# HeyWeCome/WhisprRec

Hardware: AMD Instinct MI355X
Metric: BPR training triplets/sec (higher is better)
Workload: dtype f32; 1 GPU; BPRMF emb_size=64, synthetic 1000000 users x 1000000 items (uniform ids), batch 65536, SGD l2=0, plan build in timed region; batch=65536, emb_size=64, optimizer=SGD, plan_chunk_batches=64, tables=single GPU, step_stream=whisprrec_amd.hip_ops.PipelinedSgd, plan=group plan (no per-batch sort: flags + lists of the shared rows, wr_group.hip), chained_step_launch=True, plan_build=on a side stream, beside the steps of the chunk before

## Files before the change

include/whisprrec_hip.h:

```cpp
#ifndef WHISPRREC_HIP_H
#define WHISPRREC_HIP_H

#include <stdint.h>

#ifdef __cplusplus
extern "C" {
#endif

#define WR_ABI_VERSION 1

#define WR_OK 0
#define WR_E_NULL (-1)
#define WR_E_SHAPE (-2)
#define WR_E_WORKSPACE (-3)
#define WR_E_ALIGN (-4)
#define WR_E_RANGE (-5)

int32_t wr_abi_version(void);
const char *wr_last_error(void);
int32_t wr_device_info(int32_t *n_cu, int32_t *wave_size, char *arch, int32_t arch_len);

int64_t wr_bpr_fwd_workspace_bytes(int64_t B);
int32_t wr_bpr_fwd(const float *user_tab, int64_t n_users, const float *item_tab, int64_t n_items, int32_t D,
                   const int64_t *u, const int64_t *p, const int64_t *n, int64_t B, float *pos_score, float *neg_score,
// ... 127 lines not shown
                          int64_t workspace_bytes, void *stream);

int32_t wr_bprmf_run_sgd(float *user_tab, int64_t n_users, float *item_tab, int64_t n_items, int32_t D,
                         const int32_t *tu, const int32_t *tp, const int32_t *tn, const int32_t *oc_item,
                         const int32_t *oc_src, int64_t n_triplets, int64_t batch_size, int64_t first_batch,
                         int64_t n_batches, float lr, float *loss_out, void *const *phase_events, const wr_hot_runs *hot,
                         void *workspace, int64_t workspace_bytes, void *stream);

int32_t wr_bprmf_chain_supported(const float *user_tab, const float *item_tab, int32_t D);
int64_t wr_bprmf_chain_sync_words(int64_t n_batches);
int32_t wr_bprmf_run_sgd_chain(float *user_tab, int64_t n_users, float *item_tab, int64_t n_items, int32_t D,
                               const int32_t *tu, const int32_t *tp, const int32_t *tn, const int32_t *oc_item,
                               const int32_t *oc_src, int64_t n_triplets, int64_t batch_size, int64_t first_batch,
                               int64_t n_batches, float lr, float *loss_out, const int32_t *tdef, const int32_t *def_q,
                               const int32_t *def_count_host, int64_t def_cap, int64_t def_limit, void *const *phase_events,
                               void *workspace, int64_t workspace_bytes, int32_t *sync, int64_t sync_words, void *stream);

int64_t wr_group_plan_words(int64_t n_triplets, int64_t batch_size, int64_t n_users, int64_t n_items);
int32_t wr_group_plan_layout(int64_t n_triplets, int64_t batch_size, int64_t n_users, int64_t n_items, int64_t *out);
int32_t wr_narrow_ids_i64(const int64_t *u, const int64_t *p, const int64_t *n, int32_t *u32, int32_t *p32, int32_t *n32,
                          int64_t count, void *stream);
int32_t wr_group_plan_build(const int32_t *u, const int32_t *p, const int32_t *n, int64_t n_triplets, int64_t batch_size,
                            int64_t n_users, int64_t n_items, int32_t *plan, int64_t plan_words, void *stream);
int64_t wr_bprmf_group_workspace_bytes(int64_t batch_size, int32_t D);
int64_t wr_bprmf_group_sync_words(int64_t n_batches);
int32_t wr_bprmf_group_supported(const float *user_tab, const float *item_tab, int32_t D);
int32_t wr_bprmf_run_sgd_group(float *user_tab, int64_t n_users, float *item_tab, int64_t n_items, int32_t D,
                               const int32_t *u, const int32_t *p, const int32_t *n, int64_t n_triplets, int64_t batch_size,
                               const int32_t *plan, int64_t plan_words, int64_t first_batch, int64_t n_batches, float lr,
                               float *loss_out, void *const *events, void *workspace, int64_t workspace_bytes, int32_t *sync,
                               int64_t sync_words, void *stream);

int32_t wr_bprmf_plan_overlap_marks(const int32_t *tu, const int32_t *tp, const int32_t *tn, int64_t n_triplets,
                                    int64_t batch_size, int64_t n_items, const int32_t *prev_bitmap, int32_t *bitmap,
                                    int32_t *tdef, int32_t *def_q, int64_t def_cap, int32_t *def_count, void *stream);

int32_t wr_bprmf_plan_overlap_deferred(const int32_t *tu, const int32_t *tp, const int32_t *tn, int64_t n_triplets,
                                       int64_t batch_size, int64_t n_items, const int32_t *prev_bitmap, const int32_t *bitmap,
                                       int32_t *tdef, int32_t *def_q, int64_t def_cap, int32_t *def_count, void *stream);

int32_t wr_bprmf_grads(const float *user_tab, int64_t n_users, const float *item_tab, int64_t n_items, int32_t D,
                       const int32_t *tu, const int32_t *tp, const int32_t *tn, const int32_t *oc_item,
                       const int32_t *oc_src, int64_t B, float *grad_u, float *grad_i, int32_t *stamp_u,
                       int32_t *stamp_i, int32_t step_id, float *loss_out, const wr_hot_runs *hot, void *workspace,
                       int64_t workspace_bytes, void *stream);

// ... 208 lines not shown
```

whisprrec_amd/abi.py:

```python
import ctypes
import os

_HERE = os.path.dirname(os.path.abspath(__file__))
LIB_PATH = os.path.join(_HERE, "libwhisprrec_hip.so")

c_i32, c_i64, c_f32, c_vp = ctypes.c_int32, ctypes.c_int64, ctypes.c_float, ctypes.c_void_p

SIGNATURES = {
    "wr_abi_version": (c_i32, []),
    "wr_last_error": (ctypes.c_char_p, []),
    "wr_device_info": (c_i32, [c_vp, c_vp, c_vp, c_i32]),
    "wr_bpr_fwd_workspace_bytes": (c_i64, [c_i64]),
    "wr_bpr_fwd": (c_i32, [c_vp, c_i64, c_vp, c_i64, c_i32, c_vp, c_vp, c_vp, c_i64, c_vp, c_vp, c_vp, c_vp, c_vp, c_i64,
                           c_vp]),
    "wr_bprmf_plan_workspace_bytes": (c_i64, [c_i64, c_i64, c_i64, c_i64]),
    "wr_bprmf_plan_build_i64": (c_i32, [c_vp, c_vp, c_vp, c_i64, c_i64, c_i64, c_i64, c_vp, c_vp, c_vp, c_vp, c_vp, c_vp,
                                        c_vp, c_vp, c_i64, c_vp]),
    "wr_bprmf_plan_build_i32": (c_i32, [c_vp, c_vp, c_vp, c_i64, c_i64, c_i64, c_i64, c_vp, c_vp, c_vp, c_vp, c_vp, c_vp,
                                        c_vp, c_vp, c_i64, c_vp]),
    "wr_bprmf_plan_small_max_batch": (c_i64, []),
    "wr_bprmf_plan_build_small_i64": (c_i32, [c_vp, c_vp, c_vp, c_i64, c_i64, c_i64, c_i64, c_vp, c_vp, c_vp, c_vp, c_vp, c_vp,
                                              c_vp, c_vp]),
    "wr_bprmf_plan_build_small_i32": (c_i32, [c_vp, c_vp, c_vp, c_i64, c_i64, c_i64, c_i64, c_vp, c_vp, c_vp, c_vp, c_vp, c_vp,
                                              c_vp, c_vp]),
# ... 35 lines not shown
    "wr_bprmf_hot_caps": (None, [c_i64, c_i32, c_vp, c_vp]),
    "wr_bprmf_plan_hot_runs": (c_i32, [c_vp, c_i32, c_i64, c_i64, c_vp, c_vp, c_vp, c_vp, c_vp, c_vp, c_vp]),
    "wr_bprmf_step_sgd": (c_i32, [c_vp, c_i64, c_vp, c_i64, c_i32, c_vp, c_vp, c_vp, c_vp, c_vp, c_i64, c_f32, c_f32,
                                  c_vp, c_vp, c_i32, c_vp, c_vp, c_vp, c_i64, c_vp]),
    "wr_bprmf_run_sgd": (c_i32, [c_vp, c_i64, c_vp, c_i64, c_i32, c_vp, c_vp, c_vp, c_vp, c_vp, c_i64, c_i64, c_i64,
                                 c_i64, c_f32, c_vp, c_vp, c_vp, c_vp, c_i64, c_vp]),
    "wr_bprmf_chain_supported": (c_i32, [c_vp, c_vp, c_i32]),
    "wr_bprmf_chain_sync_words": (c_i64, [c_i64]),
    "wr_bprmf_run_sgd_chain": (c_i32, [c_vp, c_i64, c_vp, c_i64, c_i32, c_vp, c_vp, c_vp, c_vp, c_vp, c_i64, c_i64, c_i64,
                                       c_i64, c_f32, c_vp, c_vp, c_vp, c_vp, c_i64, c_i64, c_vp, c_vp, c_i64, c_vp, c_i64,
                                       c_vp]),
    "wr_lightgcn_step_workspace_bytes": (c_i64, [c_i64, c_i64, c_i32, c_i64, c_i64]),
    "wr_lightgcn_step": (c_i32, [c_vp, c_vp, c_i64, c_i64, c_i32, c_i64, c_vp, c_vp, c_vp, c_vp, c_i32, c_i32, c_vp, c_vp, c_vp,
                                 c_i64, c_f32, c_i32, c_vp, c_vp, c_vp, c_vp, c_i64, c_vp]),
    "wr_shard_route": (c_i32, [c_vp, c_vp, c_vp, c_i64, c_i64, c_i32, c_i32, c_i64, c_i64, c_i64, c_i64, c_i64, c_vp, c_vp, c_vp,
                               c_vp, c_vp, c_vp, c_vp]),
    "wr_shard_pack": (c_i32, [c_vp, c_vp, c_i64, c_i32, c_i64, c_i64, c_vp, c_i64, c_vp, c_vp, c_vp]),
    "wr_bprmf_shard_step_group": (c_i32, [c_vp, c_i64, c_vp, c_i64, c_i64, c_i32, c_vp, c_vp, c_vp, c_i64, c_i64, c_vp, c_i64,
                                          c_i64, c_i64, c_f32, c_vp, c_vp, c_vp, c_i64, c_vp, c_i64, c_vp]),
    "wr_group_plan_words": (c_i64, [c_i64, c_i64, c_i64, c_i64]),
    "wr_group_plan_layout": (c_i32, [c_i64, c_i64, c_i64, c_i64, c_vp]),
    "wr_narrow_ids_i64": (c_i32, [c_vp, c_vp, c_vp, c_vp, c_vp, c_vp, c_i64, c_vp]),
    "wr_group_plan_build": (c_i32, [c_vp, c_vp, c_vp, c_i64, c_i64, c_i64, c_i64, c_vp, c_i64, c_vp]),
    "wr_bprmf_group_workspace_bytes": (c_i64, [c_i64, c_i32]),
    "wr_bprmf_group_sync_words": (c_i64, [c_i64]),
    "wr_bprmf_group_supported": (c_i32, [c_vp, c_vp, c_i32]),
    "wr_bprmf_run_sgd_group": (c_i32, [c_vp, c_i64, c_vp, c_i64, c_i32, c_vp, c_vp, c_vp, c_i64, c_i64, c_vp, c_i64, c_i64,
                                       c_i64, c_f32, c_vp, c_vp, c_vp, c_i64, c_vp, c_i64, c_vp]),
    "wr_bprmf_plan_overlap_deferred": (c_i32, [c_vp, c_vp, c_vp, c_i64, c_i64, c_i64, c_vp, c_vp, c_vp, c_vp, c_i64, c_vp,
                                               c_vp]),
    "wr_bprmf_plan_fast_marks_supported": (c_i32, [c_i64, c_i64, c_i64, c_i64]),
    "wr_bprmf_plan_build_fast_marks_i64": (c_i32, [c_vp, c_vp, c_vp, c_i64, c_i64, c_i64, c_i64, c_vp, c_vp, c_vp, c_vp, c_vp,
                                                   c_vp, c_vp, c_vp, c_i64, c_vp, c_vp]),
    "wr_bprmf_plan_build_fast_marks_i32": (c_i32, [c_vp, c_vp, c_vp, c_i64, c_i64, c_i64, c_i64, c_vp, c_vp, c_vp, c_vp, c_vp,
                                                   c_vp, c_vp, c_vp, c_i64, c_vp, c_vp]),
    "wr_bprmf_plan_overlap_marks": (c_i32, [c_vp, c_vp, c_vp, c_i64, c_i64, c_i64, c_vp, c_vp, c_vp, c_vp, c_i64, c_vp,
                                            c_vp]),
    "wr_bprmf_grads": (c_i32, [c_vp, c_i64, c_vp, c_i64, c_i32, c_vp, c_vp, c_vp, c_vp, c_vp, c_i64, c_vp, c_vp, c_vp,
                               c_vp, c_i32, c_vp, c_vp, c_vp, c_i64, c_vp]),
    "wr_sgd_decay_untouched": (c_i32, [c_vp, c_i64, c_i32, c_vp, c_i32, c_f32, c_f32, c_vp]),
    "wr_sgd_dense": (c_i32, [c_vp, c_i64, c_i32, c_vp, c_vp, c_i32, c_f32, c_f32, c_vp]),
    "wr_adam_dense": (c_i32, [c_vp, c_vp, c_vp, c_i64, c_i32, c_vp, c_vp, c_i32, c_i64, c_f32, c_f32, c_f32, c_f32,
                              c_f32, c_vp]),
    "wr_adam_dense_dev": (c_i32, [c_vp, c_vp, c_vp, c_i64, c_i32, c_vp, c_vp, c_i64, c_vp, c_f32, c_f32, c_f32, c_f32, c_vp]),
    "wr_adam_dense_dev_pair": (c_i32, [c_vp, c_vp, c_vp, c_i64, c_vp, c_vp, c_vp, c_vp, c_i64, c_vp, c_i32, c_vp, c_i64, c_vp,
                                       c_f32, c_f32, c_f32, c_f32, c_vp]),
# ... 133 lines not shown
```

whisprrec_amd/csrc/wr_group.hip:

```cpp
#include "wr_common.h"
#include <hip/hip_ext.h>

#include <algorithm>

namespace wr {

constexpr int kGpThreads = 1024;
constexpr unsigned kGpRangeBits = 18;
constexpr int kGpWords = 1 << (kGpRangeBits - 5);
constexpr int kGpCap = 8192;
constexpr int kGpBins = 4096;
constexpr int kGpMaxBin = 256;
constexpr int kGpMaxRanges = 8;
constexpr int64_t kGpMaxBatch = 1 << 17;
constexpr int kGpLongRun = 64;
constexpr int kGpMetaWords = 16;
#ifndef WR_GP_DBG
#define WR_GP_DBG 0
#endif

struct GroupLayout {
    int64_t nb, B, fw;
    int R_u, R_i, cap_u, cap_i;
    unsigned mask_u, mask_i, hbits_u, hbits_i;
    int64_t flags, ucnt, icnt, ul_row, ul_src, il_row, il_src, total;
    int64_t zero_words;
};

static inline int ranges_for(int64_t n_rows, unsigned *mask, unsigned *hbits, int *cap) {
    unsigned bits = kGpRangeBits;
    while (bits < kGpRangeBits + 3 && (int64_t(1) << bits) < n_rows) ++bits;
    *mask = (1u << bits) - 1u;
    *hbits = bits;
    const int R = 1 << (bits - kGpRangeBits);
    *cap = kGpCap;
    return R;
}

static bool group_layout(int64_t n, int64_t B, int64_t n_users, int64_t n_items, GroupLayout &L) {
    if (n <= 0 || n >= (int64_t(1) << 31) || B <= 0 || B > kGpMaxBatch) return false;
    if (n_users <= 0 || n_users >= (int64_t(1) << 31) || n_items <= 0 || n_items >= (int64_t(1) << 31)) return false;
    L.nb = (n + B - 1) / B;
    L.B = B;
    L.fw = (B + 31) / 32;
    L.R_u = ranges_for(n_users, &L.mask_u, &L.hbits_u, &L.cap_u);
    L.R_i = ranges_for(n_items, &L.mask_i, &L.hbits_i, &L.cap_i);
    L.flags = kGpMetaWords;
    L.ucnt = L.flags + L.nb * L.fw * 4;
    L.icnt = L.ucnt + align_up(L.nb * L.R_u, 4);
    L.zero_words = L.icnt + align_up(L.nb * L.R_i, 4);
    L.ul_row = L.zero_words;
    L.ul_src = L.ul_row + L.nb * L.R_u * (int64_t)L.cap_u;
    L.il_row = L.ul_src + L.nb * L.R_u * (int64_t)L.cap_u;
    L.il_src = L.il_row + L.nb * L.R_i * (int64_t)L.cap_i;
    L.total = L.il_src + L.nb * L.R_i * (int64_t)L.cap_i;
    return true;
}

struct GpDev {
    int *meta;
    unsigned *flags;
    int *ucnt, *icnt;
    int *ul_row, *ul_src, *il_row, *il_src;
    int R_u, R_i, cap_u, cap_i;
    unsigned mask_u, mask_i, hbits_u, hbits_i;
    int fw;
};

static inline GpDev group_dev(int32_t *plan, const GroupLayout &L) {
    return GpDev{plan, reinterpret_cast<unsigned *>(plan + L.flags), plan + L.ucnt, plan + L.icnt, plan + L.ul_row,
                 plan + L.ul_src, plan + L.il_row, plan + L.il_src, L.R_u, L.R_i, L.cap_u, L.cap_i, L.mask_u, L.mask_i,
                 L.hbits_u, L.hbits_i, (int)L.fw};
}

template <typename F>
__device__ __forceinline__ void gp_scan(const int *__restrict__ a, int cnt, F f) {
    if ((reinterpret_cast<uintptr_t>(a) & 15u) == 0) {
        const int n4 = cnt >> 2;
        const int4 *a4 = reinterpret_cast<const int4 *>(a);
        int i = threadIdx.x;
        for (; i + 3 * kGpThreads < n4; i += 4 * kGpThreads) {
            int4 v[4];
#pragma unroll
            for (int q = 0; q < 4; ++q) v[q] = a4[i + q * kGpThreads];
#pragma unroll
            for (int q = 0; q < 4; ++q) {
                const int at = 4 * (i + q * kGpThreads);
                f(v[q].x, at);
                f(v[q].y, at + 1);
                f(v[q].z, at + 2);
                f(v[q].w, at + 3);
            }
        }
        for (; i < n4; i += kGpThreads) {
            const int4 v = a4[i];
            f(v.x, 4 * i);
            f(v.y, 4 * i + 1);
            f(v.z, 4 * i + 2);
            f(v.w, 4 * i + 3);
        }
        for (int j = (n4 << 2) + threadIdx.x; j < cnt; j += kGpThreads) f(a[j], j);
    } else {
        for (int j = threadIdx.x; j < cnt; j += kGpThreads) f(a[j], j);
    }
}

__global__ __launch_bounds__(kGpThreads) void group_plan_kernel(const int *__restrict__ u, const int *__restrict__ p,
                                                                 const int *__restrict__ n, int64_t n_total, int B, int nb,
                                                                 int n_users, int n_items, GpDev L) {
    extern __shared__ __attribute__((aligned(16))) unsigned gp_lds[];
    unsigned *seen = gp_lds;
    unsigned long long *keys = reinterpret_cast<unsigned long long *>(gp_lds);
    unsigned *multi = gp_lds + 2 * kGpCap;
    unsigned *f0 = multi + kGpWords, *f1 = f0 + L.fw, *f2 = f1 + L.fw;
    int &n_list = *reinterpret_cast<int *>(f2 + L.fw);
    const int per = L.R_u + L.R_i;
    const unsigned lb = xcd_contiguous_id(blockIdx.x, gridDim.x);
    const int b = (int)(lb / (unsigned)per), rr = (int)(lb % (unsigned)per);
    const bool item = rr >= L.R_u;
    const unsigned r = (unsigned)(item ? rr - L.R_u : rr);
    const int64_t base = (int64_t)b * B;
    const int Bb = (int)((base + B <= n_total) ? B : (n_total - base));
    const unsigned n_rows = (unsigned)(item ? n_items : n_users);
    const unsigned mask = item ? L.mask_i : L.mask_u;
    const unsigned rb = (item ? L.hbits_i : L.hbits_u) - kGpRangeBits, rsel = (1u << rb) - 1u;
    for (int i = threadIdx.x; i < kGpWords; i += kGpThreads) {
        seen[i] = 0u;
        multi[i] = 0u;
    }
    for (int i = threadIdx.x; i < 3 * L.fw; i += kGpThreads) f0[i] = 0u;
    if (threadIdx.x == 0) n_list = 0;
    __syncthreads();
    auto mark = [&](int row, int) {
        if ((unsigned)row >= n_rows) {
            L.meta[0] = 1;
            return;
        }
        const unsigned h = (unsigned)row & mask;
        if ((h & rsel) != r) return;
        const unsigned bit = h >> rb, m = 1u << (bit & 31u);
        const unsigned old = atomicOr(&seen[bit >> 5], m);
        if (old & m) atomicOr(&multi[bit >> 5], m);
    };
    if (!(WR_GP_DBG & 8)) {
        if (item) {
            gp_scan(p + base, Bb, mark);
            gp_scan(n + base, Bb, mark);
        } else {
            gp_scan(u + base, Bb, mark);
        }
    }
    __syncthreads();
    auto several = [&](int row) -> bool {
        const unsigned h = (unsigned)row & mask;
        if ((h & rsel) != r) return false;
        const unsigned bit = h >> rb;
        return (multi[bit >> 5] >> (bit & 31u)) & 1u;
    };
    auto append = [&](int row, unsigned src) {
        const int pos = atomicAdd(&n_list, 1);
        if (pos < kGpCap) keys[pos] = ((unsigned long long)(unsigned)row << 32) | src;
    };
    if (!(WR_GP_DBG & 2)) {
        const bool next = b + 1 < nb && !(WR_GP_DBG & 16);
        const int64_t nbase = base + B;
        const int Bn = next ? (int)((nbase + B <= n_total) ? B : (n_total - nbase)) : 0;
        auto defer = [&](int row, int t) {
            if (several(row)) atomicOr(&f2[t >> 5], 1u << (t & 31));
        };
        if (item) {
            gp_scan(p + base, Bb, [&](int row, int t) {
                if (several(row)) {
                    atomicOr(&f0[t >> 5], 1u << (t & 31));
                    append(row, (unsigned)t << 1);
                }
            });
            gp_scan(n + base, Bb, [&](int row, int t) {
                if (several(row)) {
                    atomicOr(&f1[t >> 5], 1u << (t & 31));
                    append(row, ((unsigned)t << 1) | 1u);
                }
            });
            gp_scan(p + nbase, Bn, defer);
            gp_scan(n + nbase, Bn, defer);
        } else {
            gp_scan(u + base, Bb, [&](int row, int t) {
                if (several(row)) {
                    atomicOr(&f0[t >> 5], 1u << (t & 31));
                    append(row, (unsigned)t << 1);
                }
            });
            gp_scan(u + nbase, Bn, defer);
        }
// ... 54 lines not shown
            const int bin = bin_of(k);
            const int lo = bin ? cnt[bin - 1] : 0, hi = cnt[bin];
            if (hi - lo > kGpMaxBin) {
                L.meta[1] = 1;
                continue;
            }
            int pos = lo, same = 0;
            for (int jj = lo; jj < hi; ++jj) {
                const unsigned long long o = keys[out16[jj]];
                pos += o < k ? 1 : 0;
                same += (unsigned)(o >> 32) == (unsigned)(k >> 32) ? 1 : 0;
            }
            if (same > kGpLongRun) L.meta[2] = 1;
            lrow[pos] = (int)(k >> 32);
            lsrc[pos] = (int)(unsigned)k;
        }
    } else {
        for (int j = threadIdx.x; j < m; j += kGpThreads) {
            lrow[j] = (int)(keys[j] >> 32);
            lsrc[j] = (int)(unsigned)keys[j];
        }
    }
    if (threadIdx.x == 0) (item ? L.icnt : L.ucnt)[(int64_t)b * R + r] = m;
}

__global__ __launch_bounds__(kBlock) void narrow_ids_kernel(const int64_t *__restrict__ u, const int64_t *__restrict__ p,
                                                             const int64_t *__restrict__ n, int *__restrict__ u32,
                                                             int *__restrict__ p32, int *__restrict__ n32, int64_t cnt) {
    const int64_t i = (int64_t)blockIdx.x * kBlock + threadIdx.x;
    if (i >= cnt) return;
    const int64_t a = u[i], b = p[i], c = n[i];
    u32[i] = (a >= 0 && a < (int64_t(1) << 31)) ? (int)a : -1;
    p32[i] = (b >= 0 && b < (int64_t(1) << 31)) ? (int)b : -1;
    n32[i] = (c >= 0 && c < (int64_t(1) << 31)) ? (int)c : -1;
}

constexpr int kGsTile = 32;
constexpr int kGsAhead = 8;
constexpr int kGsShards = 64;
constexpr int kGsShardStride = 16;
constexpr int kGsStepWords = kGsShards * kGsShardStride;
constexpr int kGsDefChunk = 32;
constexpr int kGsLdsInts = 1024 + 8;
constexpr unsigned kGsSpinLimit = 1u << 22;

struct GsBatch {
// ... 468 lines not shown
        a.tiles_at = (int)((int64_t)a.nA * WR_GS_TILES_AT / 16);
        a.side_at = std::max(a.tiles_at, (int)((int64_t)a.nA * WR_GS_SIDE_AT / 16));
        const dim3 grid((unsigned)(a.nA + a.nIT + a.nUT + a.nDS));
        hipEvent_t e0 = have_cur ? ev(k, 0) : nullptr, e1 = have_cur ? ev(k, 1) : nullptr;
        if (e0 != nullptr || e1 != nullptr)
            hipExtLaunchKernelGGL((bprmf_group_step<T, NV, FULL>), grid, dim3(kBlock), 0, stream, e0, e1, 0, a);
        else
            hipLaunchKernelGGL((bprmf_group_step<T, NV, FULL>), grid, dim3(kBlock), 0, stream, a);
        WR_LAUNCH_CHECK("bprmf_group_step");
        n_partials_prev = a.nA + a.nDS;
    }
    return WR_OK;
}

}

using namespace wr;

extern "C" {

int64_t wr_group_plan_words(int64_t n_triplets, int64_t batch_size, int64_t n_users, int64_t n_items) {
    GroupLayout L;
    if (!group_layout(n_triplets, batch_size, n_users, n_items, L)) return 0;
    return L.total;
}

int32_t wr_group_plan_layout(int64_t n_triplets, int64_t batch_size, int64_t n_users, int64_t n_items, int64_t *out) {
    WR_REQUIRE(out != nullptr, WR_E_NULL, "out is NULL");
    GroupLayout L;
    WR_REQUIRE(group_layout(n_triplets, batch_size, n_users, n_items, L), WR_E_RANGE,
               "group plan not applicable to n=%lld, batch=%lld", (long long)n_triplets, (long long)batch_size);
    const int64_t v[16] = {L.nb, L.fw, L.R_u, L.R_i, (int64_t)L.mask_u, (int64_t)L.mask_i, L.flags, L.ucnt, L.icnt, L.ul_row,
                           L.ul_src, L.il_row, L.il_src, L.total, L.cap_u, L.cap_i};
    for (int i = 0; i < 16; ++i) out[i] = v[i];
    return WR_OK;
}

int32_t wr_narrow_ids_i64(const int64_t *u, const int64_t *p, const int64_t *n, int32_t *u32, int32_t *p32, int32_t *n32,
                          int64_t count, void *stream_) {
    WR_REQUIRE(u && p && n && u32 && p32 && n32, WR_E_NULL, "index arrays must not be NULL");
    WR_REQUIRE(count >= 0 && count < (int64_t(1) << 40), WR_E_SHAPE, "count out of range");
    if (count == 0) return WR_OK;
    hipLaunchKernelGGL(narrow_ids_kernel, dim3((unsigned)((count + kBlock - 1) / kBlock)), dim3(kBlock), 0,
                       reinterpret_cast<hipStream_t>(stream_), u, p, n, u32, p32, n32, count);
    WR_LAUNCH_CHECK("narrow_ids_kernel");
    return WR_OK;
}

int32_t wr_group_plan_build(const int32_t *u, const int32_t *p, const int32_t *n, int64_t n_triplets, int64_t batch_size,
                            int64_t n_users, int64_t n_items, int32_t *plan, int64_t plan_words, void *stream_) {
    WR_REQUIRE(u && p && n && plan, WR_E_NULL, "index arrays / plan must not be NULL");
    GroupLayout L;
    WR_REQUIRE(group_layout(n_triplets, batch_size, n_users, n_items, L), WR_E_RANGE,
               "group plan not applicable to n=%lld, batch=%lld", (long long)n_triplets, (long long)batch_size);
    WR_REQUIRE(aligned16(plan) && plan_words >= L.total, WR_E_WORKSPACE, "group plan: %lld words < %lld", (long long)plan_words,
               (long long)L.total);
    WR_REQUIRE(L.nb * (L.R_u + L.R_i) < (int64_t(1) << 31), WR_E_SHAPE, "group plan: too many batches in one plan");
    hipStream_t stream = reinterpret_cast<hipStream_t>(stream_);
    WR_HIP(hipMemsetAsync(plan, 0, (size_t)L.zero_words * 4, stream));
    const size_t lds = (size_t)(2 * kGpCap + kGpWords + 3 * L.fw + 4) * 4;
    static bool attr_set = false;
    if (!attr_set) {
        WR_HIP(hipFuncSetAttribute(reinterpret_cast<const void *>(group_plan_kernel), hipFuncAttributeMaxDynamicSharedMemorySize,
                                   (int)((2 * kGpCap + kGpWords + 3 * ((kGpMaxBatch + 31) / 32) + 4) * 4)));
        attr_set = true;
    }
    const GpDev G = group_dev(plan, L);
    hipLaunchKernelGGL(group_plan_kernel, dim3((unsigned)(L.nb * (L.R_u + L.R_i))), dim3(kGpThreads), lds, stream, u, p, n,
                       n_triplets, (int)batch_size, (int)L.nb, (int)n_users, (int)n_items, G);
    WR_LAUNCH_CHECK("group_plan_kernel");
    return WR_OK;
}

int64_t wr_bprmf_group_workspace_bytes(int64_t batch_size, int32_t D) { return 2 * gs_ws_one(batch_size, D); }

int64_t wr_bprmf_group_sync_words(int64_t n_batches) { return n_batches < 0 ? WR_E_SHAPE : (n_batches + 1) * kGsStepWords + 4; }

int32_t wr_bprmf_group_supported(const float *user_tab, const float *item_tab, int32_t D) {
    return (user_tab && item_tab && D >= 4 && D <= 1024 && D % 4 == 0 && gs_shape_ok(user_tab, item_tab, D)) ? 1 : 0;
}

int32_t wr_bprmf_run_sgd_group(float *user_tab, int64_t n_users, float *item_tab, int64_t n_items, int32_t D,
                               const int32_t *u, const int32_t *p, const int32_t *n, int64_t n_triplets, int64_t batch_size,
                               const int32_t *plan, int64_t plan_words, int64_t first_batch, int64_t n_batches, float lr,
                               float *loss_out, void *const *events, void *workspace, int64_t workspace_bytes, int32_t *sync,
                               int64_t sync_words, void *stream_) {
    int32_t rc;
    if ((rc = check_table(user_tab, n_users, D, "user_tab")) != WR_OK) return rc;
    if ((rc = check_table(item_tab, n_items, D, "item_tab")) != WR_OK) return rc;
    WR_REQUIRE(u && p && n && plan && sync, WR_E_NULL, "index arrays / plan / sync words must not be NULL");
    WR_REQUIRE(gs_shape_ok(user_tab, item_tab, D), WR_E_ALIGN,
               "wr_bprmf_run_sgd_group: rows must be whole 128-B lines (D %% 32 == 0, tables 128-B aligned); D = %d", (int)D);
    GroupLayout L;
    WR_REQUIRE(group_layout(n_triplets, batch_size, n_users, n_items, L), WR_E_RANGE,
// ... 68 lines not shown
```

whisprrec_amd/hip_ops.py:

```python
import ctypes

import torch

from . import abi


def _stream():
    return torch.cuda.current_stream().cuda_stream


def _p(t):
    return None if t is None else t.data_ptr()


def _req(t, dtype, name, ndim=None):
    if not isinstance(t, torch.Tensor):
        raise TypeError("%s must be a torch.Tensor" % name)
    if t.device.type != "cuda":
        raise abi.WhisprRecHipError("%s must live on a ROCm device (got %s); there is no CPU fallback" % (name, t.device))
    if t.dtype != dtype:
        raise TypeError("%s must be %s (got %s)" % (name, dtype, t.dtype))
    if not t.is_contiguous():
        raise ValueError("%s must be contiguous" % name)
    if ndim is not None and t.dim() != ndim:
# ... 473 lines not shown

class GroupArena:

    def __init__(self, device, max_triplets, batch_size, n_users, n_items):
        words = int(abi.lib().wr_group_plan_words(int(max_triplets), int(batch_size), int(n_users), int(n_items)))
        if words <= 0:
            raise abi.WhisprRecHipError("group plan: shape not supported (batch size %d)" % batch_size)
        self.device, self.max_triplets, self.batch_size = device, int(max_triplets), int(batch_size)
        self.n_users, self.n_items = int(n_users), int(n_items)
        self.buf = torch.empty(words, dtype=torch.int32, device=device)
        self.meta_host = torch.zeros(GroupPlan.META, dtype=torch.int32, pin_memory=True)
        self.meta_np = self.meta_host.numpy()
        self.free = None

    def release_after(self, stream):
        self.free = torch.cuda.Event()
        self.free.record(stream)


class GroupPlan:

    META = 16

    def __init__(self, u, p, n, batch_size, n_users, n_items, arena=None, defer=False):
        u, p, n = (_req(t, torch.int32, nm, 1) for t, nm in ((u, "u"), (p, "p"), (n, "n")))
        N = u.numel()
        if not (p.numel() == N and n.numel() == N) or N == 0:
            raise ValueError("u/p/n must have the same non-zero length")
        L = abi.lib()
        self.u, self.p, self.n = u, p, n
        self.n_triplets, self.batch_size = N, int(batch_size)
        self.n_users, self.n_items = int(n_users), int(n_items)
        self.n_batches = (N + self.batch_size - 1) // self.batch_size
        self.words = int(L.wr_group_plan_words(N, self.batch_size, self.n_users, self.n_items))
        if self.words <= 0:
            raise abi.WhisprRecHipError("group plan: shape not supported (batch size %d)" % self.batch_size)
        self.arena = arena
        self._stream = torch.cuda.current_stream(u.device)
        if arena is not None:
            if arena.buf.numel() < self.words or arena.batch_size != self.batch_size or \
                    (arena.n_users, arena.n_items) != (self.n_users, self.n_items):
                raise ValueError("plan does not fit its arena")
            if arena.free is not None:
                self._stream.wait_event(arena.free)
                arena.free = None
            self.buf = arena.buf
            self._pinned = arena.meta_host
        else:
            self.buf = torch.empty(self.words, dtype=torch.int32, device=u.device)
            self._pinned = None
        abi.check(L.wr_group_plan_build(_p(u), _p(p), _p(n), N, self.batch_size, self.n_users, self.n_items, _p(self.buf),
                                        self.buf.numel(), _stream()), "wr_group_plan_build")
        self.ready = None
        if self._pinned is not None:
            self._pinned.copy_(self.buf[:self.META], non_blocking=True)
            self.ready = torch.cuda.Event()
            self.ready.record(self._stream)
        self._finished = False
        self.bad_index = self.overflow = self.long_run = False
        if not defer:
            self.finish()

    def finish(self):
        if self._finished:
            return self
        if self._pinned is not None:
            self.ready.synchronize()
            m = self.arena.meta_np
        else:
            m = self.buf[:self.META].cpu().numpy()
        self.bad_index, self.overflow, self.long_run = bool(m[0]), bool(m[1]), bool(m[2])
        self._finished = True
        return self

    def finish_from(self, meta):
# ... 517 lines not shown
def adam_dense(tab, exp_avg, exp_avg_sq, grad, adam_step, lr, l2=0.0, beta1=0.9, beta2=0.999, eps=1e-8, stamp=None,
               step_id=0):
    for t, nm in ((tab, "tab"), (exp_avg, "exp_avg"), (exp_avg_sq, "exp_avg_sq"), (grad, "grad")):
        _req(t, torch.float32, nm, 2)
    abi.check(abi.lib().wr_adam_dense(_p(tab), _p(exp_avg), _p(exp_avg_sq), tab.shape[0], tab.shape[1], _p(grad),
                                      _p(stamp), step_id, adam_step, lr, l2, beta1, beta2, eps, _stream()),
              "wr_adam_dense")


def _join_views(ts):
    if len(ts) == 1:
        return ts[0]
    a = ts[0]
    adjacent, end = a.is_contiguous(), a.storage_offset() + a.numel()
    for b in ts[1:]:
        adjacent = adjacent and b.is_contiguous() and b.dtype == a.dtype and \
            b.untyped_storage().data_ptr() == a.untyped_storage().data_ptr() and b.storage_offset() == end
        end += b.numel()
    if adjacent:
        return torch.as_strided(a, (end - a.storage_offset(),), (1,), a.storage_offset())
    return torch.cat(ts)


class PipelinedSgd:

    PREFETCH_AFTER_TRIPLETS = 0
    PLAN_TRIPLETS = 1 << 22
    GROUP_MIN_ROWS_PER_TRIPLET = 12
    GROUP_MIN_BATCH = 4096

    CHAIN_MIN_BATCH = 8192
    CHAIN_MIN_ITEMS_PER_TRIPLET = 6

    def __init__(self, chunk=64, min_triplets=None, chain=True, inline_plan=False, group=True):
        import sys
        self.ops = sys.modules[__name__]
        self.chunk = int(chunk)
        self.chain = bool(chain)
        self.group = bool(group)
        self.inline_plan = inline_plan
        self.stats = {"plain_calls": 0, "chain_calls": 0, "group_calls": 0, "group_fallbacks": 0}
        self._garenas = {}
        if min_triplets is not None:
            self.PLAN_TRIPLETS = int(min_triplets)
        self.plan_stream = None
        self._arenas = {}

    def chunk_batches(self, batch_size):
        return max(self.chunk, self.PLAN_TRIPLETS // max(int(batch_size), 1))

    def _arena_pair(self, device, B, nb_total, overlap_items):
        cap = min(self.chunk_batches(B), max(int(nb_total), 1)) * B
# ... 75 lines not shown
                    abi.check(abi.lib().wr_narrow_ids_i64(*[_p(c[lo:hi]) for c in cols], *[_p(c[lo:hi]) for c in h["ids32"]],
                                                          hi - lo, _stream()), "wr_narrow_ids_i64")
                    cols = h["ids32"]
                plan = self.ops.GroupPlan(cols[0][lo:hi], cols[1][lo:hi], cols[2][lo:hi], B, h["n_users"], h["n_items"],
                                          arena=h["garenas"][h["tag"]], defer=True)
                h["tag"] ^= 1
                h["next"] = (first, plan)
                return
            if h["arenas"] is None:
                h["arenas"] = self._arena_pair(h["device"], B, h["nb"], h["n_items"] if h["chain"] else 0)
            plan = self.ops.BatchPlan(h["u"][lo:hi], h["p"][lo:hi], h["n"][lo:hi], B, h["n_users"], h["n_items"],
                                      validate=False, ws_tag="rot%d" % h["tag"], bucket_map=bmap, arena=h["arenas"][h["tag"]],
                                      defer=True, overlap=h["chain"])
        h["tag"] ^= 1
        h["next"] = (first, plan)

    STICKY_MSG = "a wait inside a step launch expired (hand-off between the workgroups of one launch): the tables are not " \
                 "valid — do not save or evaluate them; restart the run"

    def _queue_sticky(self, h, tabs, main):
        words = tabs.sticky_words()
        if not words:
            return
        pin = h.get("sticky_pin")
        if pin is None or pin.numel() < 2 * len(words):
            pin = h["sticky_pin"] = torch.zeros(2 * max(len(words), 4), dtype=torch.int32, pin_memory=True)
        half = pin.numel() // 2
        off = half * (h.get("sticky_tag", 0) & 1)
        h["sticky_tag"] = h.get("sticky_tag", 0) + 1
        for j, wd in enumerate(words):
            pin[off + j:off + j + 1].copy_(wd, non_blocking=True)
        ev = torch.cuda.Event()
        ev.record(main)
        self._check_sticky(h)
        h["sticky_pending"] = (ev, pin[off:off + len(words)])

    def _check_sticky(self, h):
        pend = h.pop("sticky_pending", None)
        if pend is not None:
            pend[0].synchronize()
            if bool(pend[1].numpy().any()):
                raise abi.WhisprRecHipError(self.STICKY_MSG)

    def _take_next(self, h, pos, main):
        self._check_sticky(h)
        if h["next"] is None:
            self._prefetch(h)
        cur = h["next"]
        assert cur is not None and cur[0] == pos, "steps must be run in order"
        plan = cur[1]
        plan.validate()
        if isinstance(plan, GroupPlan):
            if plan.overflow or plan.long_run:
                h["group"] = False
                self.stats["group_fallbacks"] += 1
                if h["next"] is not None and h["next"][0] != cur[0]:
                    raise AssertionError("plan pipeline out of step")
                if plan.overflow:
                    first, B = cur[0], h["B"]
                    lo, hi = first * B, first * B + plan.n_triplets
                    plan.arena.release_after(main)
                    if h["arenas"] is None:
                        h["arenas"] = self._arena_pair(h["device"], B, h["nb"], h["n_items"] if h["chain"] else 0)
                    with torch.cuda.stream(self._build_stream(h)):
                        plan = self.ops.BatchPlan(h["u"][lo:hi], h["p"][lo:hi], h["n"][lo:hi], B, h["n_users"], h["n_items"],
# ... 46 lines not shown
                h["runner"](plan, pos - base, c, losses[loss_off:loss_off + c])
                self.stats["plain_calls"] += 1
            elif h["chain"] and plan.overlap is not None and c >= 2:
                sg["tabs"].run_sgd_chain(plan, pos - base, c, lr, losses=losses[loss_off:loss_off + c])
                self.stats["chain_calls"] += 1
            else:
                sg["tabs"].run_sgd(plan, pos - base, c, lr, losses=losses[loss_off:loss_off + c])
                self.stats["plain_calls"] += 1
            pos += c
            loss_off += c
            if pos >= base + plan.n_batches:
                plan.arena.release_after(main)
                self._queue_sticky(h, sg["tabs"], main)
            if h["next"] is None and not h["inline"]:
                self._prefetch(h)
        h["pos"] = pos

    def run(self, handle, seg, lr, losses):
        sg = handle["segs"][seg]
        if sg["nb"] == 0:
            return
        self._run_span(handle, sg, sg["first"], sg["first"] + sg["nb"], lr, losses, 0)
        if seg == len(handle["segs"]) - 1:
            self._check_sticky(handle)

    def run_steps(self, handle, count, lr, losses):
        assert len(handle["segs"]) == 1, "run_steps: single-segment handles"
        sg = handle["segs"][0]
        pos = handle["pos"]
        if pos + count > sg["nb"]:
            raise ValueError("run_steps: %d steps asked, %d left" % (count, sg["nb"] - pos))
        self._run_span(handle, sg, pos, pos + count, lr, losses, 0)


class LazyOptimizerState:

    FOLD_MAX_GAP = 40

    MAX_LAG = 64
    LAG_MIN_GAP = 64

    def __init__(self, tabs, name, lr, l2, betas=(0.9, 0.999), eps=1e-8, fold=None, max_lag=None):
        self.chain, self.chain_calls = True, 0
        if name not in ("SGD", "Adam"):
            raise ValueError(name)
        self.tabs, self.name, self.lr, self.l2, self.betas, self.eps = tabs, name, float(lr), float(l2), betas, float(eps)
        self.fold = fold if fold is None else bool(fold)
# ... 500 lines not shown
```

Baseline: 2.721 billion triplets/s.

## Add single-visit group plan build with dealt buckets and deeper sticky readbacks

Adds a single-visit group-plan variant. A deal kernel splits each batch's ids into per-range buckets, so each plan workgroup scans only its own bucket instead of the whole batch. It also lets several sticky-error readbacks be outstanding instead of blocking on the previous one each chunk. The single-visit path is compiled off by default (WR_GP_SINGLE_VISIT=0) and the Python caller never passes single_visit, so only the sticky readback change runs by default. The plan buffer also grows to hold the bucket slots.

```diff
diff --git a/include/whisprrec_hip.h b/include/whisprrec_hip.h
--- a/include/whisprrec_hip.h
+++ b/include/whisprrec_hip.h
@@ -173,6 +173,9 @@
                           int64_t count, void *stream);
 int32_t wr_group_plan_build(const int32_t *u, const int32_t *p, const int32_t *n, int64_t n_triplets, int64_t batch_size,
                             int64_t n_users, int64_t n_items, int32_t *plan, int64_t plan_words, void *stream);
+int32_t wr_group_plan_build_variant(const int32_t *u, const int32_t *p, const int32_t *n, int64_t n_triplets, int64_t batch_size,
+                                    int64_t n_users, int64_t n_items, int32_t *plan, int64_t plan_words, int32_t single_visit,
+                                    void *stream);
 int64_t wr_bprmf_group_workspace_bytes(int64_t batch_size, int32_t D);
 int64_t wr_bprmf_group_sync_words(int64_t n_batches);
 int32_t wr_bprmf_group_supported(const float *user_tab, const float *item_tab, int32_t D);
diff --git a/whisprrec_amd/abi.py b/whisprrec_amd/abi.py
--- a/whisprrec_amd/abi.py
+++ b/whisprrec_amd/abi.py
@@ -81,6 +81,7 @@
     "wr_group_plan_layout": (c_i32, [c_i64, c_i64, c_i64, c_i64, c_vp]),
     "wr_narrow_ids_i64": (c_i32, [c_vp, c_vp, c_vp, c_vp, c_vp, c_vp, c_i64, c_vp]),
     "wr_group_plan_build": (c_i32, [c_vp, c_vp, c_vp, c_i64, c_i64, c_i64, c_i64, c_vp, c_i64, c_vp]),
+    "wr_group_plan_build_variant": (c_i32, [c_vp, c_vp, c_vp, c_i64, c_i64, c_i64, c_i64, c_vp, c_i64, c_i32, c_vp]),
     "wr_bprmf_group_workspace_bytes": (c_i64, [c_i64, c_i32]),
     "wr_bprmf_group_sync_words": (c_i64, [c_i64]),
     "wr_bprmf_group_supported": (c_i32, [c_vp, c_vp, c_i32]),
diff --git a/whisprrec_amd/csrc/wr_group.hip b/whisprrec_amd/csrc/wr_group.hip
--- a/whisprrec_amd/csrc/wr_group.hip
+++ b/whisprrec_amd/csrc/wr_group.hip
@@ -15,6 +15,13 @@
 constexpr int64_t kGpMaxBatch = 1 << 17;
 constexpr int kGpLongRun = 64;
 constexpr int kGpMetaWords = 16;
+constexpr int kGpDealBits = 14;
+constexpr int kGpDeal = 1 << kGpDealBits;
+constexpr int kGpMaxChunks = 8;
+constexpr int kGpPass = 64;
+#ifndef WR_GP_SINGLE_VISIT
+#define WR_GP_SINGLE_VISIT 0
+#endif
 #ifndef WR_GP_DBG
 #define WR_GP_DBG 0
 #endif
@@ -25,6 +32,8 @@
     unsigned mask_u, mask_i, hbits_u, hbits_i;
     int64_t flags, ucnt, icnt, ul_row, ul_src, il_row, il_src, total;
     int64_t zero_words;
+    int nC, S, sub_u, sub_i;
+    int64_t slot_cnt, slot_words, bk_cnt, bk, alloc;
 };
 
 static inline int ranges_for(int64_t n_rows, unsigned *mask, unsigned *hbits, int *cap) {
@@ -54,6 +63,17 @@
     L.il_row = L.ul_src + L.nb * L.R_u * (int64_t)L.cap_u;
     L.il_src = L.il_row + L.nb * L.R_i * (int64_t)L.cap_i;
     L.total = L.il_src + L.nb * L.R_i * (int64_t)L.cap_i;
+    const int deal = (int)std::min<int64_t>(kGpDeal, align_up(B, 4));
+    auto sub_of = [&](int R) { return R == 1 ? deal : (int)std::min<int64_t>(deal, align_up(deal / R * 3 / 2 + 64, 4)); };
+    L.nC = (int)((B + kGpDeal - 1) / kGpDeal);
+    L.S = (int)std::min<int64_t>(L.nb, kGpPass + 1);
+    L.sub_u = sub_of(L.R_u);
+    L.sub_i = sub_of(L.R_i);
+    L.slot_cnt = align_up((int64_t)L.nC * (L.R_u + 2 * L.R_i), 4);
+    L.slot_words = (int64_t)L.nC * ((int64_t)L.R_u * L.sub_u + 2 * (int64_t)L.R_i * L.sub_i);
+    L.bk_cnt = align_up(L.total, 4);
+    L.bk = L.bk_cnt + L.S * L.slot_cnt;
+    L.alloc = L.bk + L.S * L.slot_words;
     return true;
 }
 
@@ -65,12 +85,24 @@
     int R_u, R_i, cap_u, cap_i;
     unsigned mask_u, mask_i, hbits_u, hbits_i;
     int fw;
+    int *bk_cnt;
+    unsigned *bk;
+    int nC, S, sub_u, sub_i, slot_cnt, slot_words;
 };
 
 static inline GpDev group_dev(int32_t *plan, const GroupLayout &L) {
     return GpDev{plan, reinterpret_cast<unsigned *>(plan + L.flags), plan + L.ucnt, plan + L.icnt, plan + L.ul_row,
                  plan + L.ul_src, plan + L.il_row, plan + L.il_src, L.R_u, L.R_i, L.cap_u, L.cap_i, L.mask_u, L.mask_i,
-                 L.hbits_u, L.hbits_i, (int)L.fw};
+                 L.hbits_u, L.hbits_i, (int)L.fw, plan + L.bk_cnt, reinterpret_cast<unsigned *>(plan + L.bk), L.nC, L.S, L.sub_u,
+                 L.sub_i, (int)L.slot_cnt, (int)L.slot_words};
+}
+
+__device__ __forceinline__ unsigned *gp_bucket(const GpDev &L, int slot, int col, int c, unsigned r, int *&cnt) {
+    const int R = col ? L.R_i : L.R_u, sub = col ? L.sub_i : L.sub_u;
+    const int64_t col_words = col ? (int64_t)L.nC * L.R_u * L.sub_u + (int64_t)(col - 1) * L.nC * L.R_i * L.sub_i : 0;
+    const int col_cnt = col ? L.nC * L.R_u + (col - 1) * L.nC * L.R_i : 0;
+    cnt = L.bk_cnt + (int64_t)slot * L.slot_cnt + col_cnt + c * R + (int)r;
+    return L.bk + (int64_t)slot * L.slot_words + col_words + ((int64_t)c * R + r) * sub;
 }
 
 template <typename F>
@@ -105,18 +137,47 @@
     }
 }
 
+template <typename F>
+__device__ __forceinline__ void gp_scan_bucket(const unsigned *__restrict__ a, int cnt, int col, int c, F f) {
+    const int n4 = cnt >> 2;
+    const uint4 *a4 = reinterpret_cast<const uint4 *>(a);
+    int i = threadIdx.x;
+    for (; i + 3 * kGpThreads < n4; i += 4 * kGpThreads) {
+        uint4 v[4];
+#pragma unroll
+        for (int q = 0; q < 4; ++q) v[q] = a4[i + q * kGpThreads];
+#pragma unroll
+        for (int q = 0; q < 4; ++q) {
+            f(v[q].x, col, c);
+            f(v[q].y, col, c);
+            f(v[q].z, col, c);
+            f(v[q].w, col, c);
+        }
+    }
+    for (; i < n4; i += kGpThreads) {
+        const uint4 v = a4[i];
+        f(v.x, col, c);
+        f(v.y, col, c);
+        f(v.z, col, c);
+        f(v.w, col, c);
+    }
+    for (int j = (n4 << 2) + threadIdx.x; j < cnt; j += kGpThreads) f(a[j], col, c);
+}
+
+template <bool SV>
 __global__ __launch_bounds__(kGpThreads) void group_plan_kernel(const int *__restrict__ u, const int *__restrict__ p,
                                                                  const int *__restrict__ n, int64_t n_total, int B, int nb,
-                                                                 int n_users, int n_items, GpDev L) {
+                                                                 int b0, int n_users, int n_items, GpDev L) {
     extern __shared__ __attribute__((aligned(16))) unsigned gp_lds[];
     unsigned *seen = gp_lds;
     unsigned long long *keys = reinterpret_cast<unsigned long long *>(gp_lds);
     unsigned *multi = gp_lds + 2 * kGpCap;
     unsigned *f0 = multi + kGpWords, *f1 = f0 + L.fw, *f2 = f1 + L.fw;
     int &n_list = *reinterpret_cast<int *>(f2 + L.fw);
+    int *sub_cnt = reinterpret_cast<int *>(f2 + L.fw) + 4;
     const int per = L.R_u + L.R_i;
     const unsigned lb = xcd_contiguous_id(blockIdx.x, gridDim.x);
-    const int b = (int)(lb / (unsigned)per), rr = (int)(lb % (unsigned)per);
+    const int b = b0 + (int)(lb / (unsigned)per), rr = (int)(lb % (unsigned)per);
     const bool item = rr >= L.R_u;
     const unsigned r = (unsigned)(item ? rr - L.R_u : rr);
     const int64_t base = (int64_t)b * B;
@@ -130,6 +191,27 @@
     }
     for (int i = threadIdx.x; i < 3 * L.fw; i += kGpThreads) f0[i] = 0u;
     if (threadIdx.x == 0) n_list = 0;
+    const bool has_next = b + 1 < nb && !(WR_GP_DBG & 16);
+    const int col0 = item ? 1 : 0, n_cols = item ? 2 : 1;
+    const bool hashed = n_rows > mask + 1u;
+    if constexpr (SV) {
+        const int j = (int)threadIdx.x, which = j / (2 * kGpMaxChunks), k = j % (2 * kGpMaxChunks);
+        if (which < 2 && k < n_cols * L.nC) {
+            int *cp = nullptr;
+            if (which == 0 || has_next) gp_bucket(L, (b + which) % L.S, col0 + k / L.nC, k % L.nC, r, cp);
+            sub_cnt[j] = cp ? min(max(*cp, 0), item ? L.sub_i : L.sub_u) : 0;
+        }
+    }
+    const int Rs = item ? L.R_i : L.R_u, subs = item ? L.sub_i : L.sub_u, n_bk = n_cols * L.nC, nC = L.nC;
+    const unsigned *bk_cur = nullptr, *bk_next = nullptr;
+    if constexpr (SV) {
+        int *cp;
+        bk_cur = gp_bucket(L, b % L.S, col0, 0, r, cp);
+        bk_next = gp_bucket(L, (b + 1) % L.S, col0, 0, r, cp);
+    }
+    auto buckets = [&](const unsigned *bk, const int *cnts, auto f) __attribute__((always_inline)) {
+        for (int k = 0; k < n_bk; ++k) gp_scan_bucket(bk + (int64_t)k * Rs * subs, cnts[k], col0 + k / nC, k % nC, f);
+    };
     __syncthreads();
     auto mark = [&](int row, int) {
         if ((unsigned)row >= n_rows) {
@@ -143,7 +225,13 @@
         if (old & m) atomicOr(&multi[bit >> 5], m);
     };
     if (!(WR_GP_DBG & 8)) {
-        if (item) {
+        if constexpr (SV) {
+            buckets(bk_cur, sub_cnt, [&](unsigned e, int, int) {
+                const unsigned bit = e >> kGpDealBits, m = 1u << (bit & 31u);
+                const unsigned old = atomicOr(&seen[bit >> 5], m);
+                if (old & m) atomicOr(&multi[bit >> 5], m);
+            });
+        } else if (item) {
             gp_scan(p + base, Bb, mark);
             gp_scan(n + base, Bb, mark);
         } else {
@@ -168,7 +256,27 @@
         auto defer = [&](int row, int t) {
             if (several(row)) atomicOr(&f2[t >> 5], 1u << (t & 31));
         };
-        if (item) {
+        if constexpr (SV) {
+            int *nl = &n_list;
+            buckets(bk_cur, sub_cnt, [u, p, n, f0, f1, multi, keys, nl, base, rb, r, hashed](unsigned e, int col, int c) {
+                const unsigned bit = e >> kGpDealBits;
+                if (!((multi[bit >> 5] >> (bit & 31u)) & 1u)) return;
+                const int t = (c << kGpDealBits) | (int)(e & (kGpDeal - 1));
+                atomicOr(&(col == 2 ? f1 : f0)[t >> 5], 1u << (t & 31));
+                int row = (int)((bit << rb) | r);
+                if (hashed) row = (col == 0 ? u : (col == 1 ? p : n))[base + t];
+                const int pos = atomicAdd(nl, 1);
+                if (pos < kGpCap) keys[pos] = ((unsigned long long)(unsigned)row << 32) | ((unsigned)t << 1) | (col == 2 ? 1u : 0u);
+            });
+            if (has_next)
+                buckets(bk_next, sub_cnt + 2 * kGpMaxChunks, [&](unsigned e, int, int c) {
+                    const unsigned bit = e >> kGpDealBits;
+                    if ((multi[bit >> 5] >> (bit & 31u)) & 1u) {
+                        const int t = (c << kGpDealBits) | (int)(e & (kGpDeal - 1));
+                        atomicOr(&f2[t >> 5], 1u << (t & 31));
+                    }
+                });
+        } else if (item) {
             gp_scan(p + base, Bb, [&](int row, int t) {
                 if (several(row)) {
                     atomicOr(&f0[t >> 5], 1u << (t & 31));
@@ -269,6 +377,65 @@
         }
     }
     if (threadIdx.x == 0) (item ? L.icnt : L.ucnt)[(int64_t)b * R + r] = m;
+}
+
+__global__ __launch_bounds__(kGpThreads) void group_deal_kernel(const int *__restrict__ u, const int *__restrict__ p,
+                                                                 const int *__restrict__ n, int64_t n_total, int B, int b0,
+                                                                 int n_users, int n_items, GpDev L) {
+    extern __shared__ __attribute__((aligned(16))) unsigned gp_lds[];
+    int *lcnt = reinterpret_cast<int *>(gp_lds);
+    const int per = 3 * L.nC;
+    const int b = b0 + (int)(blockIdx.x / (unsigned)per), rem = (int)(blockIdx.x % (unsigned)per);
+    const int col = rem / L.nC, c = rem % L.nC;
+    const bool item = col > 0;
+    const int64_t base = (int64_t)b * B;
+    const int Bb = (int)((base + B <= n_total) ? B : (n_total - base));
+    const int len = max(0, min(kGpDeal, Bb - (c << kGpDealBits)));
+    const int *ids = (col == 0 ? u : (col == 1 ? p : n)) + base + ((int64_t)c << kGpDealBits);
+    const unsigned n_rows = (unsigned)(item ? n_items : n_users);
+    const unsigned mask = item ? L.mask_i : L.mask_u;
+    const unsigned rb = (item ? L.hbits_i : L.hbits_u) - kGpRangeBits, rsel = (1u << rb) - 1u;
+    const int R = item ? L.R_i : L.R_u, sub = item ? L.sub_i : L.sub_u;
+    int *cnt_out;
+    unsigned *bk = gp_bucket(L, b % L.S, col, c, 0u, cnt_out);
+    if (threadIdx.x < kGpMaxRanges) lcnt[threadIdx.x] = 0;
+    __syncthreads();
+    const int lane = (int)(threadIdx.x & 63u);
+    constexpr int kU = 4;
+    for (int j0 = 0; j0 < len; j0 += kU * kGpThreads) {
+        int row[kU];
+#pragma unroll
+        for (int q = 0; q < kU; ++q) {
+            const int j = j0 + q * kGpThreads + (int)threadIdx.x;
+            row[q] = j < len ? ids[j] : 0;
+        }
+#pragma unroll
+        for (int q = 0; q < kU; ++q) {
+            const int j = j0 + q * kGpThreads + (int)threadIdx.x;
+            const bool valid = j < len;
+            if (valid && (unsigned)row[q] >= n_rows) L.meta[0] = 1;
+            const unsigned h = (unsigned)row[q] & mask, rr = h & rsel;
+            unsigned long long mine = 0ull;
+            for (int k = 0; k < R; ++k) {
+                const unsigned long long mk = __ballot(valid && rr == (unsigned)k);
+                if (rr == (unsigned)k) mine = mk;
+            }
+            const int rank = __popcll(mine & ((1ull << lane) - 1ull));
+            int at = 0;
+            if (valid && rank == 0) at = atomicAdd(&lcnt[rr], __popcll(mine));
+            at = __shfl(at, valid ? __ffsll((long long)mine) - 1 : lane, 64) + rank;
+            if (valid && at < sub) bk[(int64_t)rr * sub + at] = ((h >> rb) << kGpDealBits) | (unsigned)j;
+        }
+    }
+    __syncthreads();
+    if ((int)threadIdx.x < R) {
+        int m = lcnt[threadIdx.x];
+        if (m > sub) {
+            L.meta[1] = 1;
+            m = sub;
+        }
+        cnt_out[threadIdx.x] = m;
+    }
 }
 
 __global__ __launch_bounds__(kBlock) void narrow_ids_kernel(const int64_t *__restrict__ u, const int64_t *__restrict__ p,
@@ -783,7 +950,7 @@
 int64_t wr_group_plan_words(int64_t n_triplets, int64_t batch_size, int64_t n_users, int64_t n_items) {
     GroupLayout L;
     if (!group_layout(n_triplets, batch_size, n_users, n_items, L)) return 0;
-    return L.total;
+    return L.alloc;
 }
 
 int32_t wr_group_plan_layout(int64_t n_triplets, int64_t batch_size, int64_t n_users, int64_t n_items, int64_t *out) {
@@ -808,29 +975,56 @@
     return WR_OK;
 }
 
-int32_t wr_group_plan_build(const int32_t *u, const int32_t *p, const int32_t *n, int64_t n_triplets, int64_t batch_size,
-                            int64_t n_users, int64_t n_items, int32_t *plan, int64_t plan_words, void *stream_) {
+int32_t wr_group_plan_build_variant(const int32_t *u, const int32_t *p, const int32_t *n, int64_t n_triplets, int64_t batch_size,
+                                    int64_t n_users, int64_t n_items, int32_t *plan, int64_t plan_words, int32_t single_visit,
+                                    void *stream_) {
     WR_REQUIRE(u && p && n && plan, WR_E_NULL, "index arrays / plan must not be NULL");
     GroupLayout L;
     WR_REQUIRE(group_layout(n_triplets, batch_size, n_users, n_items, L), WR_E_RANGE,
                "group plan not applicable to n=%lld, batch=%lld", (long long)n_triplets, (long long)batch_size);
-    WR_REQUIRE(aligned16(plan) && plan_words >= L.total, WR_E_WORKSPACE, "group plan: %lld words < %lld", (long long)plan_words,
-               (long long)L.total);
+    WR_REQUIRE(aligned16(plan) && plan_words >= L.alloc, WR_E_WORKSPACE, "group plan: %lld words < %lld", (long long)plan_words,
+               (long long)L.alloc);
     WR_REQUIRE(L.nb * (L.R_u + L.R_i) < (int64_t(1) << 31), WR_E_SHAPE, "group plan: too many batches in one plan");
     hipStream_t stream = reinterpret_cast<hipStream_t>(stream_);
     WR_HIP(hipMemsetAsync(plan, 0, (size_t)L.zero_words * 4, stream));
-    const size_t lds = (size_t)(2 * kGpCap + kGpWords + 3 * L.fw + 4) * 4;
+    const size_t lds = (size_t)(2 * kGpCap + kGpWords + 3 * L.fw + 4 + 4 * kGpMaxChunks) * 4;
     static bool attr_set = false;
     if (!attr_set) {
-        WR_HIP(hipFuncSetAttribute(reinterpret_cast<const void *>(group_plan_kernel), hipFuncAttributeMaxDynamicSharedMemorySize,
-                                   (int)((2 * kGpCap + kGpWords + 3 * ((kGpMaxBatch + 31) / 32) + 4) * 4)));
+        const int max_lds = (int)((2 * kGpCap + kGpWords + 3 * ((kGpMaxBatch + 31) / 32) + 4 + 4 * kGpMaxChunks) * 4);
+        WR_HIP(hipFuncSetAttribute(reinterpret_cast<const void *>(group_plan_kernel<false>),
+                                   hipFuncAttributeMaxDynamicSharedMemorySize, max_lds));
+        WR_HIP(hipFuncSetAttribute(reinterpret_cast<const void *>(group_plan_kernel<true>),
+                                   hipFuncAttributeMaxDynamicSharedMemorySize, max_lds));
         attr_set = true;
     }
     const GpDev G = group_dev(plan, L);
-    hipLaunchKernelGGL(group_plan_kernel, dim3((unsigned)(L.nb * (L.R_u + L.R_i))), dim3(kGpThreads), lds, stream, u, p, n,
-                       n_triplets, (int)batch_size, (int)L.nb, (int)n_users, (int)n_items, G);
-    WR_LAUNCH_CHECK("group_plan_kernel");
+    const int per = L.R_u + L.R_i;
+    if (!single_visit) {
+        hipLaunchKernelGGL(group_plan_kernel<false>, dim3((unsigned)(L.nb * per)), dim3(kGpThreads), lds, stream, u, p, n,
+                           n_triplets, (int)batch_size, (int)L.nb, 0, (int)n_users, (int)n_items, G);
+        WR_LAUNCH_CHECK("group_plan_kernel");
+        return WR_OK;
+    }
+    for (int64_t g0 = 0; g0 < L.nb; g0 += kGpPass) {
+        const int64_t g1 = std::min<int64_t>(L.nb, g0 + kGpPass);
+        const int64_t d0 = g0 == 0 ? 0 : g0 + 1, d1 = std::min<int64_t>(g1, L.nb - 1);
+        if (d1 >= d0) {
+            hipLaunchKernelGGL(group_deal_kernel, dim3((unsigned)((d1 - d0 + 1) * 3 * L.nC)), dim3(kGpThreads),
+                               (size_t)kGpMaxRanges * 4, stream, u, p, n, n_triplets, (int)batch_size, (int)d0, (int)n_users,
+                               (int)n_items, G);
+            WR_LAUNCH_CHECK("group_deal_kernel");
+        }
+        hipLaunchKernelGGL(group_plan_kernel<true>, dim3((unsigned)((g1 - g0) * per)), dim3(kGpThreads), lds, stream, u, p, n,
+                           n_triplets, (int)batch_size, (int)L.nb, (int)g0, (int)n_users, (int)n_items, G);
+        WR_LAUNCH_CHECK("group_plan_kernel");
+    }
     return WR_OK;
+}
+
+int32_t wr_group_plan_build(const int32_t *u, const int32_t *p, const int32_t *n, int64_t n_triplets, int64_t batch_size,
+                            int64_t n_users, int64_t n_items, int32_t *plan, int64_t plan_words, void *stream_) {
+    return wr_group_plan_build_variant(u, p, n, n_triplets, batch_size, n_users, n_items, plan, plan_words, WR_GP_SINGLE_VISIT,
+                                       stream_);
 }
 
 int64_t wr_bprmf_group_workspace_bytes(int64_t batch_size, int32_t D) { return 2 * gs_ws_one(batch_size, D); }
diff --git a/whisprrec_amd/hip_ops.py b/whisprrec_amd/hip_ops.py
--- a/whisprrec_amd/hip_ops.py
+++ b/whisprrec_amd/hip_ops.py
@@ -519,7 +519,7 @@
 
     META = 16
 
-    def __init__(self, u, p, n, batch_size, n_users, n_items, arena=None, defer=False):
+    def __init__(self, u, p, n, batch_size, n_users, n_items, arena=None, defer=False, single_visit=None):
         u, p, n = (_req(t, torch.int32, nm, 1) for t, nm in ((u, "u"), (p, "p"), (n, "n")))
         N = u.numel()
         if not (p.numel() == N and n.numel() == N) or N == 0:
@@ -546,8 +546,13 @@
         else:
             self.buf = torch.empty(self.words, dtype=torch.int32, device=u.device)
             self._pinned = None
-        abi.check(L.wr_group_plan_build(_p(u), _p(p), _p(n), N, self.batch_size, self.n_users, self.n_items, _p(self.buf),
-                                        self.buf.numel(), _stream()), "wr_group_plan_build")
+        if single_visit is None:
+            abi.check(L.wr_group_plan_build(_p(u), _p(p), _p(n), N, self.batch_size, self.n_users, self.n_items, _p(self.buf),
+                                            self.buf.numel(), _stream()), "wr_group_plan_build")
+        else:
+            abi.check(L.wr_group_plan_build_variant(_p(u), _p(p), _p(n), N, self.batch_size, self.n_users, self.n_items,
+                                                    _p(self.buf), self.buf.numel(), 1 if single_visit else 0, _stream()),
+                      "wr_group_plan_build_variant")
         self.ready = None
         if self._pinned is not None:
             self._pinned.copy_(self.buf[:self.META], non_blocking=True)
@@ -1111,12 +1116,58 @@
     return torch.cat(ts)
 
 
+class StickyReadbacks:
+
+    def __init__(self, depth, message):
+        self.depth = max(int(depth), 1)
+        self.message = message
+        self.pending = []
+        self.busy = set()
+
+    def take_slot(self):
+        while len(self.busy) >= self.depth:
+            self._consume(0, wait=True)
+        slot = min(s for s in range(self.depth) if s not in self.busy)
+        self.busy.add(slot)
+        return slot
+
+    def push(self, event, slot, read):
+        assert slot in self.busy and all(p[1] != slot for p in self.pending), "slot reused before its word was read"
+        self.pending.append((event, slot, read))
+
+    def _consume(self, i, wait):
+        event, slot, read = self.pending[i]
+        if wait:
+            event.synchronize()
+        is_set = bool(read())
+        del self.pending[i]
+        self.busy.discard(slot)
+        if is_set:
+            raise abi.WhisprRecHipError(self.message)
+
+    def before_chunk(self):
+        i = 0
+        while i < len(self.pending):
+            if self.pending[i][0].query():
+                self._consume(i, wait=False)
+            else:
+                i += 1
+        while len(self.pending) >= self.depth:
+            self._consume(0, wait=True)
+
+    def drain(self):
+        while self.pending:
+            self._consume(0, wait=True)
+
+
 class PipelinedSgd:
 
     PREFETCH_AFTER_TRIPLETS = 0
     PLAN_TRIPLETS = 1 << 22
     GROUP_MIN_ROWS_PER_TRIPLET = 12
     GROUP_MIN_BATCH = 4096
+
+    STICKY_OUTSTANDING = 2
 
     CHAIN_MIN_BATCH = 8192
     CHAIN_MIN_ITEMS_PER_TRIPLET = 6
@@ -1238,25 +1289,30 @@
         words = tabs.sticky_words()
         if not words:
             return
+        st = h.get("sticky")
+        if st is None:
+            st = h["sticky"] = StickyReadbacks(self.STICKY_OUTSTANDING, self.STICKY_MSG)
         pin = h.get("sticky_pin")
-        if pin is None or pin.numel() < 2 * len(words):
-            pin = h["sticky_pin"] = torch.zeros(2 * max(len(words), 4), dtype=torch.int32, pin_memory=True)
-        half = pin.numel() // 2
-        off = half * (h.get("sticky_tag", 0) & 1)
-        h["sticky_tag"] = h.get("sticky_tag", 0) + 1
+        if pin is None or pin.numel() // st.depth < len(words):
+            st.drain()
+            pin = h["sticky_pin"] = torch.zeros(st.depth * max(len(words), 4), dtype=torch.int32, pin_memory=True)
+        width = pin.numel() // st.depth
+        slot = st.take_slot()
+        off = slot * width
         for j, wd in enumerate(words):
             pin[off + j:off + j + 1].copy_(wd, non_blocking=True)
         ev = torch.cuda.Event()
         ev.record(main)
-        self._check_sticky(h)
-        h["sticky_pending"] = (ev, pin[off:off + len(words)])
-
-    def _check_sticky(self, h):
-        pend = h.pop("sticky_pending", None)
-        if pend is not None:
-            pend[0].synchronize()
-            if bool(pend[1].numpy().any()):
-                raise abi.WhisprRecHipError(self.STICKY_MSG)
+        view = pin[off:off + len(words)].numpy()
+        st.push(ev, slot, lambda: bool(view.any()))
+
+    def _check_sticky(self, h, drain=False):
+        st = h.get("sticky")
+        if st is not None:
+            if drain:
+                st.drain()
+            else:
+                st.before_chunk()
 
     def _take_next(self, h, pos, main):
         self._check_sticky(h)
@@ -1349,7 +1405,7 @@
             return
         self._run_span(handle, sg, sg["first"], sg["first"] + sg["nb"], lr, losses, 0)
         if seg == len(handle["segs"]) - 1:
-            self._check_sticky(handle)
+            self._check_sticky(handle, drain=True)
 
     def run_steps(self, handle, count, lr, losses):
         assert len(handle["segs"]) == 1, "run_steps: single-segment handles"
```

Result: no change. 2.748 billion triplets/s, median of 6 (+1.0%).
